# davidtweedle/gptq-svd

Hardware: AMD Instinct MI355X
Metric: weight-cols quantized/sec at d_in=4096 (higher is better)
Workload: dtype f64+f32; 1 GPU; single synthetic 4096x4096 Hessian per rank, full solver (eigh, rank rule, pivot order, U, 4-bit asym g128 quantize, pack); n=4096, m=4096, calib_rows=3072, rank_k=3058, threshold_method=energy, block_size=1024, parallelism=independent layer per rank x1

## Files before the change

### gptq-svd_amd/csrc/pivot.hip

```cpp
#include <algorithm>
#include <climits>
#include <cmath>
#include <cstdio>
#include <cstdlib>
#include <type_traits>
#include <utility>

#include "../../include/truncgptq.h"
#include "common.h"
#include "spin.h"
#include "gemm64.h"
#include "reduce.h"

namespace {

constexpr int PB = 32;
constexpr int PGMAX = 64;

struct PivWs {
  double *B;
  double *Hk;
  double *dsc;
  double *L;
  double *LT;
  double *part;
  int32_t *perm;
  int32_t *pos;
  unsigned *cnt;
  double *pp;
  double *bc;
  unsigned *flag;
  int32_t *sstate;
  int32_t *prow;
  double *pinv;
  double *Lpp;
  double *Hk2;
  int32_t *oidx;
};
constexpr int PPS = PB + 8;
static_assert(PGMAX * PPS % 256 == 0, "slot copy assumes whole rounds of 256 threads");

inline bool compact_pivot(int n) { return n <= 32768 && getenv("TG_PIVOT_OLD") == nullptr; }

template <class A>
void piv_layout(A &ar, int n, int k, PivWs *p) {
  PivWs d{};
  PivWs &q = p ? *p : d;
  auto take = [&](auto *&dst, size_t cnt) {
    using T = std::remove_reference_t<decltype(*dst)>;
    if constexpr (std::is_same_v<A, tg::Arena>) dst = ar.template take<T>(cnt);
    else ar.template take<T>(cnt);
  };
  auto take2m = [&](double *&dst, size_t cnt) {
    constexpr size_t AL = size_t(2) << 20;
    if constexpr (std::is_same_v<A, tg::Arena>) dst = ar.template take_aligned<double>(cnt, AL);
    else ar.template take_aligned<double>(cnt, AL);
  };
  take(q.B, size_t(k) * n);
  take(q.pp, size_t(2) * PGMAX * PPS);
  take(q.bc, PPS);
  take(q.flag, 16);
  take2m(q.Hk, size_t(n) * n);
  take(q.dsc, n);
  take(q.L, size_t(n) * k);
  take(q.LT, size_t(PB) * n);
  take(q.part, PGMAX * 2);
  take(q.perm, n);
  take(q.pos, n);
  take(q.cnt, 16);
  take(q.sstate, 16);
  take(q.prow, PB);
  take(q.pinv, PB);
  take(q.Lpp, PB * PB);
  take2m(q.Hk2, compact_pivot(n) ? size_t(n) * n : size_t(1));
  take(q.oidx, n);
}

__global__ void scale_rows_kernel(const double *__restrict__ Vh, int ldv, const double *__restrict__ S,
                                  int n, int k, double *__restrict__ B) {
  const int t = blockIdx.y;
  const double s = S[t];
  for (int c = blockIdx.x * blockDim.x + threadIdx.x; c < n; c += gridDim.x * blockDim.x)
    B[size_t(t) * n + c] = s * Vh[size_t(t) * ldv + c];
}

__device__ inline void argmax_publish(double bv, int bp, int i, int n, PivWs w) {
  __shared__ double sv[256];
  __shared__ int sp[256];
  __shared__ double vals[2];
  const int tid = threadIdx.x;
  sv[tid] = bv;
  sp[tid] = bp;
  __syncthreads();
  for (int off = 128; off > 0; off >>= 1) {
    if (tid < off) {
      const double ov = sv[tid + off];
      const int op = sp[tid + off];
      if (ov > sv[tid] || (ov == sv[tid] && op < sp[tid])) {
        sv[tid] = ov;
        sp[tid] = op;
      }
    }
    __syncthreads();
  }
  if (tid == 0) {
    vals[0] = sv[0];
    vals[1] = double(sp[0]);
  }
  __syncthreads();
  if (tg::publish_partials(vals, 2, w.part, w.cnt)) {
    if (tid < 64) {
      const int G = int(gridDim.x);
      double best = -INFINITY;
      int q = n;
      for (int g = tid; g < G; g += 64) {
        const double v = tg::load_partial(&w.part[g]);
        const int p = int(tg::load_partial(&w.part[G + g]));
        if (v > best || (v == best && p < q)) {
          best = v;
          q = p;
        }
      }
#pragma unroll
      for (int off = 32; off > 0; off >>= 1) {
        const double ov = __shfl_xor(best, off);
        const int op = __shfl_xor(q, off);
        if (ov > best || (ov == best && op < q)) {
          best = ov;
          q = op;
        }
      }
      if (tid == 0) {
        if (q < n && q != i) {
          const int a = w.perm[i], b = w.perm[q];
          w.perm[i] = b;
          w.perm[q] = a;
          w.pos[b] = i;
          w.pos[a] = q;
        }
        *w.cnt = 0u;
      }
    }
  }
}

__global__ __launch_bounds__(256) void piv_init_kernel(int n, PivWs w) {
  double bv = -INFINITY;
  int bp = n;
  for (int j = blockIdx.x * blockDim.x + threadIdx.x; j < n; j += gridDim.x * blockDim.x) {
    const double v = w.Hk[size_t(j) * n + j];
    w.dsc[j] = v;
    w.perm[j] = j;
    w.pos[j] = j;
    if (v > bv || (v == bv && j < bp)) {
      bv = v;
      bp = j;
    }
  }
// ... 249 lines not shown
    if (tid <= t) lrow[tid] = win[8 + tid];
    const int rowb = min(max(int(win[2]), 0), n - 1);
#pragma unroll
    for (int u = 0; u < RPT; ++u) hv[u] = w.Hk[size_t(rowb) * n + min(rows[u], n - 1)];
    const int a = permL[i + 1];
    __syncthreads();
    if (tid == 0 && q != i + 1) {
      permL[i + 1] = rowb;
      permL[q] = a;
      if (me == 0) {
        w.perm[i + 1] = rowb;
        w.perm[q] = a;
        w.pos[rowb] = i + 1;
        w.pos[a] = q;
      }
    }
#pragma unroll
    for (int u = 0; u < RPT; ++u) {
      if (rows[u] == rowb) posr[u] = i + 1;
      else if (rows[u] == a && q != i + 1) posr[u] = q;
    }
    dpiv = s_best;
    piv = rowb;
    __syncthreads();
  }
  const int pw = min(pe, k) - ps;
#pragma unroll
  for (int u = 0; u < RPT; ++u) {
    const int r = rows[u];
    if (r >= n) continue;
    w.dsc[r] = dsr[u];
#pragma unroll
    for (int l = 0; l < PB; ++l) {
      if (l < pw) {
        w.L[size_t(r) * k + ps + l] = lr[u][l];
        w.LT[size_t(l) * n + r] = lr[u][l];
      }
    }
  }
}

constexpr int SEL = 1024;
constexpr int SEL_LDS_N = 8192;

#ifdef TG_SEL_PHASES
__device__ unsigned long long g_selph[16];
#define SELT(i)                                                     \
  {                                                                 \
    const uint64_t tt = __builtin_amdgcn_s_memtime();               \
    if (i > 0 && threadIdx.x == 0) atomicAdd(g_selph + i - 1, tt - selt_last); \
    selt_last = tt;                                                 \
  }
#else
#define SELT(i)
#endif

__device__ inline unsigned long long dkey(double d) {
  return d > 0.0 ? static_cast<unsigned long long>(__double_as_longlong(d)) : 0ull;
}

__device__ __forceinline__ size_t hk_at(int a, int b, int n) {
  return size_t(max(a, b)) * n + min(a, b);
}

__device__ __forceinline__ unsigned hk_at32(int a, int b, int n) {
  return unsigned(max(a, b)) * unsigned(n) + unsigned(min(a, b));
}

constexpr int STH = 512;

constexpr int NLEV = 3;
constexpr int LEV_DOWN = 8;
enum { SS_LEV = 2, SS_RUN = 3, SS_PANELS = 4, SS_EARLY = 5, SS_ESC = 6, SS_NLEV = 7, SS_NEED = 10 };
static_assert(SS_NLEV + NLEV <= SS_NEED && SS_NEED + NLEV - 1 <= 16, "sstate words");

__device__ __forceinline__ bool lev_pays(int rem, int lost) {
  const int r = rem >> 6, extra_us = 35 + r * r / 94, gain_us = 14;
  return lost * extra_us < PB * gain_us;
}

struct SelPanel {
  int n, k, ps, pe, nset, bp, brow, bo, lev;
  bool adaptive;
  double tau, bv;
  const double *dS;
  const int32_t *pS;
  int *permL;
  const int *cand;
  double2 *rec;
  int *reco;
  double *lrow;
  unsigned long long t0;
};
template <int NW, int CP>
__device__ __forceinline__ void sel_steps(const SelPanel &sp, PivWs w,
                                          const double *__restrict__ Hc);

__device__ inline double vmax_d(double a, double b) {
  double r;
  asm("v_max_f64 %0, %1, %2" : "=v"(r) : "v"(a), "v"(b));
  return r;
}
__device__ inline double sel_pair_max(double x, bool half16) {
  const int lo = __double2loint(x), hi = __double2hiint(x);
  if (half16) {
    const auto l = __builtin_amdgcn_permlane16_swap(lo, lo, false, false);
    const auto h = __builtin_amdgcn_permlane16_swap(hi, hi, false, false);
    return vmax_d(__hiloint2double(h[0], l[0]), __hiloint2double(h[1], l[1]));
  }
  const auto l = __builtin_amdgcn_permlane32_swap(lo, lo, false, false);
  const auto h = __builtin_amdgcn_permlane32_swap(hi, hi, false, false);
  return vmax_d(__hiloint2double(h[0], l[0]), __hiloint2double(h[1], l[1]));
}
template <int CTRL>
__device__ inline double sel_dpp(double x) {
  return __hiloint2double(__builtin_amdgcn_update_dpp(0, __double2hiint(x), CTRL, 0xF, 0xF, false),
                          __builtin_amdgcn_update_dpp(0, __double2loint(x), CTRL, 0xF, 0xF, false));
}
__device__ inline double wave_max_d(double x) {
  x = sel_pair_max(x, false);
  x = sel_pair_max(x, true);
  x = vmax_d(x, sel_dpp<0x140>(x));
  x = vmax_d(x, sel_dpp<0x141>(x));
  x = vmax_d(x, sel_dpp<0x1B>(x));
  return vmax_d(x, sel_dpp<0xB1>(x));
}
template <int S>
__device__ inline int wave_min_stage(int x) {
  return min(x, partner<S>(x));
}
template <int NW>
__device__ inline void block_argmax_sel(double &v, int &p, int &r, int &o, double2 *rec,
                                        int *reco) {
  const double m = wave_max_d(v);
  const bool hold = v == m;
  const unsigned long long b = __ballot(hold);
  int L = __ffsll(static_cast<long long>(b)) - 1;
  if (__popcll(b) > 1 && m != -INFINITY) {
    int pp = hold ? p : INT_MAX;
    pp = wave_min_stage<0>(pp);
    pp = wave_min_stage<1>(pp);
    pp = wave_min_stage<2>(pp);
    pp = wave_min_stage<3>(pp);
    pp = wave_min_stage<4>(pp);
    pp = wave_min_stage<5>(pp);
    L = __ffsll(static_cast<long long>(__ballot(hold & (p == pp)))) - 1;
  }
  const int wp = __builtin_amdgcn_readlane(p, L), wr = __builtin_amdgcn_readlane(r, L);
  const int wo = __builtin_amdgcn_readlane(o, L);
  if ((threadIdx.x & 63) == 0) {
    rec[threadIdx.x >> 6] = make_double2(m, __hiloint2double(wp, wr));
    reco[threadIdx.x >> 6] = wo;
  }
  __syncthreads();
  double2 x[NW];
#pragma unroll
  for (int q = 0; q < NW; ++q) x[q] = rec[q];
  v = x[0].x;
#pragma unroll
  for (int q = 1; q < NW; ++q) v = vmax_d(v, x[q].x);
  p = INT_MAX;
  r = 0;
  o = 0;
#pragma unroll
  for (int q = 0; q < NW; ++q) {
    const int op = __double2hiint(x[q].y);
    const bool take = (x[q].x == v) & (op < p);
    p = take ? op : p;
    r = take ? __double2loint(x[q].y) : r;
    o = take ? reco[q] : o;
  }
}

constexpr int HPAD = 2048 + 64;
__device__ inline int hidx(int b) { return b + (b >> 5); }

__device__ inline void hist_add_agg(unsigned *hist, int bin, bool ok, int lane) {
  unsigned long long pend = __ballot(ok);
  while (pend) {
    const int L = __ffsll(static_cast<long long>(pend)) - 1;
    const int b = __builtin_amdgcn_readlane(bin, L);
    const unsigned long long same = __ballot(ok & (bin == b));
    if (lane == L) atomicAdd(&hist[hidx(b)], unsigned(__popcll(same)));
    pend &= ~same;
  }
}

__device__ inline void hist_scan(const unsigned *hist, int target, int *out) {
  const int lane = threadIdx.x & 63, blk = 63 - lane;
  int c[32];
#pragma unroll
  for (int j = 0; j < 32; ++j) c[j] = int(hist[blk * 33 + 31 - j]);
  int sum = 0;
#pragma unroll
  for (int j = 0; j < 32; ++j) sum += c[j];
  int pre = sum;
#pragma unroll
  for (int off = 1; off < 64; off <<= 1) {
    const int o = __shfl_up(pre, off);
    pre += lane >= off ? o : 0;
  }
  int acc = pre - sum;
  if (acc < target && pre >= target) {
    int cb = 0, cbefore = 0;
    bool found = false;
#pragma unroll
    for (int j = 0; j < 32; ++j) {
      const bool hit = !found & (acc + c[j] >= target);
      cb = hit ? j : cb;
      cbefore = hit ? acc : cbefore;
      found = found | hit;
      acc += c[j];
    }
    out[0] = blk * 32 + 31 - cb;
    out[1] = cbefore;
  }
}

__global__ __launch_bounds__(STH) void piv_sel_kernel(int n, int k, PivWs w,
                                                      const double *__restrict__ Hc, int flev) {
  extern __shared__ int permL[];
  __shared__ unsigned hist[HPAD];
  __shared__ int cand[SEL + 1];
  __shared__ double2 rec[STH / 64];
  __shared__ int reco[STH / 64];
  __shared__ double sv[STH / 64];
  __shared__ int scnt[STH / 64];
  __shared__ int sel[4];
  __shared__ double lrow[PB];
  const int tid = threadIdx.x, lane = tid & 63, wid = tid >> 6;
  const int ps = w.sstate[0];
  if (ps >= k) {
    if (tid == 0) w.sstate[1] = 0;
    return;
  }
  const int pe = min(ps + PB, k);
  const int lev = flev >= 0              ? flev
                  : !lev_pays(n - ps, 1) ? NLEV - 1
                                         : min(max(w.sstate[SS_LEV], 0), NLEV - 1);
  const int nsel = SEL >> (NLEV - 1 - lev);
#ifdef TG_SEL_PHASES
  uint64_t selt_last = 0;
#endif
  SELT(0)
  int nset, bp, brow, bo;
  double tau, bv;
  const double *dS;
  const int32_t *pS;
  const bool staged = n <= SEL_LDS_N;
  double *dsh = reinterpret_cast<double *>(permL + ((n + 1) & ~1));
  int *posh = reinterpret_cast<int *>(dsh + n);
  if (staged) {
    for (int r0 = tid; r0 < n; r0 += 8 * STH) {
      double dv[8];
      int pv[8], mv[8];
#pragma unroll
      for (int u = 0; u < 8; ++u) {
        const int r = min(r0 + u * STH, n - 1);
        dv[u] = w.dsc[r];
        pv[u] = w.pos[r];
        mv[u] = w.perm[r];
      }
#pragma unroll
      for (int u = 0; u < 8; ++u)
        if (r0 + u * STH < n) {
          dsh[r0 + u * STH] = dv[u];
          posh[r0 + u * STH] = pv[u];
          permL[r0 + u * STH] = mv[u];
        }
    }
  } else {
    for (int x = tid; x < n; x += STH) permL[x] = w.perm[x];
  }
  for (int x = tid; x < HPAD; x += STH) hist[x] = 0u;
  if (tid == 0) {
    sel[0] = -1;
    sel[2] = -1;
  }
  __syncthreads();
  SELT(9)
  dS = staged ? dsh : w.dsc;
  pS = staged ? posh : w.pos;
  int valid = 0;
  for (int r0 = tid; r0 < n; r0 += 8 * STH) {
    double dv[8];
    int pv[8];
#pragma unroll
    for (int u = 0; u < 8; ++u) {
      const int r = min(r0 + u * STH, n - 1);
      dv[u] = dS[r];
      pv[u] = pS[r];
    }
#pragma unroll
    for (int u = 0; u < 8; ++u) {
      const unsigned long long key = dkey(dv[u]);
      const bool ok = (r0 + u * STH < n) & (pv[u] >= ps) & (key != 0ull);
      valid += ok;
      hist_add_agg(hist, int(key >> 52), ok, lane);
    }
  }
#pragma unroll
  for (int off = 32; off > 0; off >>= 1) valid += __shfl_xor(valid, off);
  if (lane == 0) scnt[wid] = valid;
  __syncthreads();
  valid = 0;
#pragma unroll
  for (int q = 0; q < STH / 64; ++q) valid += scnt[q];
  SELT(10)
  if (valid > nsel) {
    if (wid == 0) hist_scan(hist, nsel, sel);
    __syncthreads();
    for (int x = tid; x < HPAD; x += STH) hist[x] = 0u;
    __syncthreads();
    const int b1 = sel[0];
    for (int r0 = tid; r0 < n; r0 += 8 * STH) {
      double dv[8];
      int pv[8];
#pragma unroll
      for (int u = 0; u < 8; ++u) {
        const int r = min(r0 + u * STH, n - 1);
        dv[u] = dS[r];
        pv[u] = pS[r];
      }
#pragma unroll
      for (int u = 0; u < 8; ++u) {
        const unsigned long long key = dkey(dv[u]);
        if ((r0 + u * STH < n) & (pv[u] >= ps) & (int(key >> 52) == b1))
          atomicAdd(&hist[hidx(int(key >> 41) & 2047)], 1u);
      }
    }
    __syncthreads();
    if (wid == 0) hist_scan(hist, nsel - sel[1], sel + 2);
    __syncthreads();
  }
  SELT(11)
  const int b1 = sel[0], b2 = sel[2];
  int mine = 0;
  tau = -INFINITY;
  bv = -INFINITY;
  bp = n;
  brow = 0;
  unsigned long long insm = 0ull;
  for (int r0 = tid, bi = 0; r0 < n; r0 += 8 * STH, bi += 8) {
    double dv[8];
    int pv[8];
#pragma unroll
    for (int u = 0; u < 8; ++u) {
      const int r = min(r0 + u * STH, n - 1);
      dv[u] = dS[r];
      pv[u] = pS[r];
    }
#pragma unroll
    for (int u = 0; u < 8; ++u) {
      const bool un = (r0 + u * STH < n) & (pv[u] >= ps);
      const unsigned long long key = dkey(dv[u]);
      const int d1 = int(key >> 52), d2 = int(key >> 41) & 2047;
      const bool ins = un & (key != 0ull) & ((b1 < 0) | (d1 > b1) | ((d1 == b1) & (d2 > b2)));
      mine += ins;
      insm |= static_cast<unsigned long long>(ins) << (bi + u);
      tau = (un & !ins) ? fmax(tau, dv[u]) : tau;
      const bool take = un & ((dv[u] > bv) | ((dv[u] == bv) & (pv[u] < bp)));
      bv = take ? dv[u] : bv;
      bp = take ? pv[u] : bp;
      brow = take ? r0 + u * STH : brow;
    }
  }
  {
    int pre = mine;
#pragma unroll
    for (int off = 1; off < 64; off <<= 1) {
      const int o = __shfl_up(pre, off);
      pre += lane >= off ? o : 0;
    }
    double t2 = tau;
#pragma unroll
    for (int off = 32; off > 0; off >>= 1) t2 = fmax(t2, __shfl_xor(t2, off));
    __syncthreads();
    if (lane == 63) scnt[wid] = pre;
    if (lane == 0) sv[wid] = t2;
    __syncthreads();
    int base = 0;
    tau = -INFINITY;
#pragma unroll
    for (int q = 0; q < STH / 64; ++q) {
      base += q < wid ? scnt[q] : 0;
      tau = fmax(tau, sv[q]);
    }
    int slot = base + pre - mine;
    for (int r0 = tid, bi = 0; r0 < n; r0 += 8 * STH, bi += 8) {
#pragma unroll
      for (int u = 0; u < 8; ++u) {
        const bool ins = (insm >> (bi + u)) & 1ull;
        cand[ins ? slot : SEL] = r0 + u * STH;
        slot += ins;
      }
    }
  }
  __syncthreads();
  SELT(12)
  nset = 0;
#pragma unroll
  for (int q = 0; q < STH / 64; ++q) nset += scnt[q];
  bo = bp - ps;
  block_argmax_sel<STH / 64>(bv, bp, brow, bo, rec, reco);
  SelPanel sp{n,   k,  ps, pe,    nset, bp,   brow, bo,   lev,  flev < 0,
              tau, bv, dS, pS,    permL, cand, rec,  reco, lrow,
#ifdef TG_SEL_PHASES
              selt_last
#else
              0
#endif
  };
  if (lev == NLEV - 1) {
    sel_steps<STH / 64, 2>(sp, w, Hc);
    return;
  }
  if (wid >= 4) return;
  if (lev == 1) sel_steps<4, 2>(sp, w, Hc);
  else sel_steps<4, 1>(sp, w, Hc);
}

template <int NW, int CP>
__device__ __forceinline__ void sel_steps(const SelPanel &sp, PivWs w,
                                          const double *__restrict__ Hc) {
  constexpr int NT = NW * 64;
  const int tid = threadIdx.x;
  const int n = sp.n, k = sp.k, ps = sp.ps, pe = sp.pe, nset = sp.nset;
  const double tau = sp.tau;
  const double *dS = sp.dS;
  const int32_t *pS = sp.pS;
  int *permL = sp.permL;
  const int *cand = sp.cand;
  double2 *rec = sp.rec;
  int *reco = sp.reco;
  double *lrow = sp.lrow;
#ifdef TG_SEL_PHASES
  uint64_t selt_last = sp.t0;
#endif
  const int ss_run = w.sstate[SS_RUN], ss_esc = w.sstate[SS_ESC], ss_panels = w.sstate[SS_PANELS],
            ss_early = w.sstate[SS_EARLY], ss_nlev = w.sstate[SS_NLEV + sp.lev],
            ss_need_up = w.sstate[SS_NEED + min(sp.lev, NLEV - 2)],
            ss_need_dn = w.sstate[SS_NEED + max(sp.lev - 1, 0)];
  int rc[CP], posc[CP], oc[CP];
  double dc[CP];
  bool done[CP];
  double lr[CP][PB];
#pragma unroll
  for (int u = 0; u < CP; ++u) {
    const int c = tid + u * NT;
    rc[u] = c < nset ? cand[c] : -1;
    posc[u] = rc[u] >= 0 ? pS[rc[u]] : n;
    oc[u] = rc[u] >= 0 ? posc[u] - ps : 0;
    dc[u] = rc[u] >= 0 ? dS[rc[u]] : -INFINITY;
    done[u] = rc[u] < 0;
#pragma unroll
    for (int l = 0; l < PB; ++l) lr[u][l] = 0.0;
  }
  int piv = sp.brow, q = sp.bp, opiv = sp.bo;
  double dpiv = sp.bv;
  int tdone = 0;
  SELT(1)
  bool active = true;
  auto step = [&]<int t>(std::integral_constant<int, t>) __attribute__((always_inline)) {
    const int i = ps + t;
    active = active && i < pe;
    if (!active) return;
    if (t > 0) {
      double v = -INFINITY;
      int p = n, r = -1, o = 0;
#pragma unroll
      for (int u = 0; u < CP; ++u) {
        const bool take = !done[u] & ((dc[u] > v) | ((dc[u] == v) & (posc[u] < p)));
        v = take ? dc[u] : v;
        p = take ? posc[u] : p;
        r = take ? rc[u] : r;
        o = take ? oc[u] : o;
      }
      SELT(4)
      block_argmax_sel<NW>(v, p, r, o, rec, reco);
      SELT(5)
      active = v > tau;
      if (!active) return;
      dpiv = v;
      q = p;
      piv = r;
      opiv = o;
    }
    double hv[CP];
#pragma unroll
    for (int u = 0; u < CP; ++u)
      hv[u] = Hc[hk_at32(opiv, oc[u], n)];
#pragma unroll
    for (int u = 0; u < CP; ++u)
      if (rc[u] == piv) {
#pragma unroll
        for (int l = 0; l < t; ++l) lrow[l] = lr[u][l];
      }
    if (tid == 0) {
      const int a = permL[i];
      if (q != i) {
        permL[i] = piv;
        permL[q] = a;
      }
      w.prow[t] = piv;
    }
    SELT(2)
    __syncthreads();
    SELT(3)
    const double ljj = sqrt(fmax(dpiv, 0.0));
    const double inv = ljj > 0.0 ? 1.0 / ljj : 0.0;
    if (tid == 0) w.pinv[t] = inv;
    if (tid <= t) w.Lpp[t * PB + tid] = tid < t ? lrow[tid] : ljj;
    double lrw[PB > 1 ? PB : 1];
#pragma unroll
    for (int l = 0; l < t; ++l) lrw[l] = lrow[l];
#pragma unroll
    for (int u = 0; u < CP; ++u) {
      const bool isp = rc[u] == piv;
      const bool upd = !done[u] & !isp;
      double v = hv[u];
#pragma unroll
      for (int l = 0; l < t; ++l) v = fma(-lr[u][l], lrw[l], v);
      const double lv = v * inv;
      lr[u][t] = isp ? ljj : (upd ? lv : lr[u][t]);
      dc[u] = upd ? fma(-lv, lv, dc[u]) : dc[u];
      const int pswap = ((posc[u] == i) & (q != i)) ? q : posc[u];
      posc[u] = isp ? i : (upd ? pswap : posc[u]);
      done[u] = done[u] | isp;
    }
    tdone = t + 1;
#ifdef TG_SEL_PHASES
    if (tid == 0) atomicAdd(g_selph + 15, 1ull);
#endif
  };
  [&]<int... Ts>(std::integer_sequence<int, Ts...>) __attribute__((always_inline)) {
    (step(std::integral_constant<int, Ts>{}), ...);
  }(std::make_integer_sequence<int, PB>{});
  SELT(6)
  __syncthreads();
  for (int x = ps + tid; x < n; x += NT) w.oidx[x - ps] = pS[permL[x]] - ps;
  __syncthreads();
  for (int x = tid; x < n; x += NT) {
    const int r = permL[x];
    w.perm[x] = r;
    w.pos[r] = x;
  }
  if (tid == 0) {
    w.sstate[0] = ps + tdone;
    w.sstate[1] = tdone;
    const bool early = tdone < PB && ps + tdone < k;
    if (sp.adaptive) {
      const bool shorted = early && !lev_pays(n - ps, pe - ps - tdone);
      int lev = sp.lev, run = shorted ? 0 : ss_run + 1;
      if (shorted && lev < NLEV - 1) {
        w.sstate[SS_NEED + lev] = min(2 * max(ss_need_up, LEV_DOWN), 1 << 20);
        ++lev;
        w.sstate[SS_ESC] = ss_esc + 1;
      } else if (lev > 0 && run >= max(ss_need_dn, LEV_DOWN)) {
        --lev;
        run = 0;
      }
      w.sstate[SS_LEV] = lev;
      w.sstate[SS_RUN] = run;
    }
    w.sstate[SS_PANELS] = ss_panels + 1;
    w.sstate[SS_EARLY] = ss_early + early;
    w.sstate[SS_NLEV + sp.lev] = ss_nlev + 1;
  }
}

template <int FT>
__global__ __launch_bounds__(FT) void piv_fill_kernel(int n, int k, PivWs w,
                                                      const double *__restrict__ Hc) {
  __shared__ double lpp[PB][PB + 1];
  __shared__ double pinv[PB];
  __shared__ int prow[PB], poi[PB];
  __shared__ double lst[FT][PB + 1];
  __shared__ int rst[FT];
  const int tid = threadIdx.x;
  const int tn = w.sstate[1];
  if (tn <= 0) return;
  const int ps = w.sstate[0] - tn, ps2 = ps + tn;
  for (int x = tid; x < PB * PB; x += FT) {
    const int i = x / PB, l = x % PB;
    lpp[i][l] = (i < tn && l <= i) ? w.Lpp[x] : 0.0;
  }
  if (tid < PB) {
    pinv[tid] = tid < tn ? w.pinv[tid] : 0.0;
    prow[tid] = tid < tn ? w.prow[tid] : -1;
    poi[tid] = tid < tn ? w.oidx[tid] : 0;
  }
  __syncthreads();
  const int x = ps + blockIdx.x * FT + tid;
  const bool valid = x < n;
  const int xc = valid ? x : n - 1;
  const int r = w.perm[xc], oi = w.oidx[xc - ps];
  double hv[PB];
#pragma unroll
  for (int i = 0; i < PB; ++i) hv[i] = i < tn ? Hc[hk_at(poi[i], oi, n)] : 0.0;
  double d = w.dsc[r];
  double lr[PB];
  bool done = false;
#pragma unroll
  for (int i = 0; i < PB; ++i) {
    double v = hv[i];
#pragma unroll
    for (int l = 0; l < i; ++l) v = fma(-lr[l], lpp[i][l], v);
    const double lv = v * pinv[i];
    const bool act = (i < tn) & !done, isp = prow[i] == r;
    lr[i] = act ? (isp ? lpp[i][i] : lv) : 0.0;
    d = (act & !isp) ? fma(-lv, lv, d) : d;
    done = done | (act & isp);
  }
  if (valid) w.dsc[r] = d;
#pragma unroll
  for (int l = 0; l < PB; ++l) {
    if (valid && x >= ps2) w.LT[size_t(l) * n + (x - ps2)] = lr[l];
    lst[tid][l] = lr[l];
  }
  rst[tid] = valid ? r : -1;
  __syncthreads();
  const int hw = tid >> 5, l = tid & 31;
  for (int t = hw; t < FT; t += FT / 32) {
    const int rr = rst[t];
    if (rr >= 0 && l < tn) w.L[size_t(rr) * k + ps + l] = lst[t][l];
  }
}

typedef double doublex4 __attribute__((ext_vector_type(4)));

__global__ __launch_bounds__(256) void syrk_compact_kernel(int n, PivWs w,
                                                           const double *__restrict__ Hc,
                                                           double *__restrict__ Hn) {
  __shared__ double li[PB][64], lj[PB][64];
  __shared__ int orow[64], ocol[64];
  const int tid = threadIdx.x;
  const int ps2 = w.sstate[0], tn = max(w.sstate[1], 0);
  const int nc = n - ps2;
  const int b = blockIdx.x;
  int I = int((sqrt(8.0 * b + 1.0) - 1.0) * 0.5);
  while ((I + 1) * (I + 2) / 2 <= b) ++I;
  while (I * (I + 1) / 2 > b) --I;
  const int J = b - I * (I + 1) / 2;
  const int i0 = 64 * I, j0 = 64 * J;
  if (i0 >= nc) return;
  if (tid < 64) {
    orow[tid] = w.oidx[tn + min(i0 + tid, nc - 1)];
  } else if (tid < 128) {
    ocol[tid - 64] = w.oidx[tn + min(j0 + tid - 64, nc - 1)];
  }
  for (int e = tid; e < PB * 64; e += 256) {
    const int l = e >> 6, c = e & 63;
    li[l][c] = w.LT[size_t(l) * n + min(i0 + c, nc - 1)];
    lj[l][c] = w.LT[size_t(l) * n + min(j0 + c, nc - 1)];
  }
  __syncthreads();
  const int lane = tid & 63, wid = tid >> 6, wm = wid >> 1, wn = wid & 1;
  const int lr = lane & 15, lk = lane >> 4;
  doublex4 acc[2][2];
#pragma unroll
  for (int ib = 0; ib < 2; ++ib)
#pragma unroll
    for (int jb = 0; jb < 2; ++jb)
#pragma unroll
      for (int q = 0; q < 4; ++q)
        acc[ib][jb][q] = Hc[hk_at(orow[wm * 32 + ib * 16 + lk + 4 * q], ocol[wn * 32 + jb * 16 + lr], n)];
#pragma unroll
  for (int kq = 0; kq < PB; kq += 4) {
    double af[2], bf[2];
#pragma unroll
    for (int ib = 0; ib < 2; ++ib) af[ib] = -li[kq + lk][wm * 32 + ib * 16 + lr];
#pragma unroll
    for (int jb = 0; jb < 2; ++jb) bf[jb] = lj[kq + lk][wn * 32 + jb * 16 + lr];
#pragma unroll
    for (int ib = 0; ib < 2; ++ib)
#pragma unroll
      for (int jb = 0; jb < 2; ++jb)
        acc[ib][jb] = __builtin_amdgcn_mfma_f64_16x16x4f64(af[ib], bf[jb], acc[ib][jb], 0, 0, 0);
  }
#pragma unroll
  for (int ib = 0; ib < 2; ++ib)
#pragma unroll
    for (int jb = 0; jb < 2; ++jb)
#pragma unroll
      for (int q = 0; q < 4; ++q) {
        const int rl = wm * 32 + ib * 16 + lk + 4 * q, cl = wn * 32 + jb * 16 + lr;
        const int gi = i0 + rl, gj = j0 + cl;
        if (gi < nc && gj < nc && gi >= gj) Hn[size_t(gi) * n + gj] = acc[ib][jb][q];
      }
}

__global__ __launch_bounds__(256, 2) void syrk_compact_p_kernel(int n, PivWs w,
                                                                const double *__restrict__ Hc,
                                                                double *__restrict__ Hn) {
  __shared__ double li[PB][64], lj[PB][64];
  const int tid = threadIdx.x;
  const int ps2 = w.sstate[0], tn = max(w.sstate[1], 0);
  const int nc = n - ps2;
  if (nc <= 0) return;
  const int ntile = tg::cdiv(nc, 64), tiles = ntile * (ntile + 1) / 2;
  const int lane = tid & 63, wid = tid >> 6, wm = wid >> 1, wn = wid & 1;
  const int lr = lane & 15, lk = lane >> 4;
  auto tile_ij = [&](int b, int &i0, int &j0) __attribute__((always_inline)) {
// ... 17 lines not shown
      __attribute__((always_inline)) {
#pragma unroll
    for (int ib = 0; ib < 2; ++ib)
#pragma unroll
      for (int jb = 0; jb < 2; ++jb)
#pragma unroll
        for (int q = 0; q < 4; ++q) o[ib][jb][q] = Hc[hk_at(ro[ib][q], co[jb], n)];
  };
  int b = blockIdx.x;
  if (b >= tiles) return;
  int ro[2][4], co[2];
  double old[2][2][4], nold[2][2][4];
  load_idx(b, ro, co);
  load_old(ro, co, old);
  const int G = int(gridDim.x);
  if (b + G < tiles) load_idx(b + G, ro, co);
  for (; b < tiles; b += G) {
    int i0, j0;
    tile_ij(b, i0, j0);
    __syncthreads();
    double lv[8][2];
#pragma unroll
    for (int u = 0; u < 8; ++u) {
      const int e = tid + u * 256, l = e >> 6, c = e & 63;
      lv[u][0] = w.LT[size_t(l) * n + min(i0 + c, nc - 1)];
      lv[u][1] = w.LT[size_t(l) * n + min(j0 + c, nc - 1)];
    }
    __builtin_amdgcn_sched_barrier(0);
    const bool more = b + G < tiles;
    if (more) load_old(ro, co, nold);
    __builtin_amdgcn_sched_barrier(0);
#pragma unroll
    for (int u = 0; u < 8; ++u) {
      const int e = tid + u * 256, l = e >> 6, c = e & 63;
      li[l][c] = lv[u][0];
      lj[l][c] = lv[u][1];
    }
    __syncthreads();
    if (b + 2 * G < tiles) load_idx(b + 2 * G, ro, co);
    doublex4 acc[2][2];
#pragma unroll
    for (int ib = 0; ib < 2; ++ib)
#pragma unroll
      for (int jb = 0; jb < 2; ++jb)
#pragma unroll
        for (int q = 0; q < 4; ++q) acc[ib][jb][q] = old[ib][jb][q];
#pragma unroll
    for (int kq = 0; kq < PB; kq += 4) {
      double af[2], bf[2];
#pragma unroll
      for (int ib = 0; ib < 2; ++ib) af[ib] = -li[kq + lk][wm * 32 + ib * 16 + lr];
#pragma unroll
      for (int jb = 0; jb < 2; ++jb) bf[jb] = lj[kq + lk][wn * 32 + jb * 16 + lr];
#pragma unroll
      for (int ib = 0; ib < 2; ++ib)
#pragma unroll
        for (int jb = 0; jb < 2; ++jb)
          acc[ib][jb] = __builtin_amdgcn_mfma_f64_16x16x4f64(af[ib], bf[jb], acc[ib][jb], 0, 0, 0);
    }
#pragma unroll
    for (int ib = 0; ib < 2; ++ib)
#pragma unroll
      for (int jb = 0; jb < 2; ++jb)
#pragma unroll
        for (int q = 0; q < 4; ++q) {
          const int rl = wm * 32 + ib * 16 + lk + 4 * q, cl = wn * 32 + jb * 16 + lr;
          const int gi = i0 + rl, gj = j0 + cl;
          if (gi < nc && gj < nc && gi >= gj) Hn[size_t(gi) * n + gj] = acc[ib][jb][q];
        }
#pragma unroll
    for (int ib = 0; ib < 2; ++ib)
#pragma unroll
      for (int jb = 0; jb < 2; ++jb)
#pragma unroll
        for (int q = 0; q < 4; ++q) old[ib][jb][q] = nold[ib][jb][q];
  }
}

__global__ __launch_bounds__(256) void piv_init2_kernel(int n, PivWs w) {
  for (int j = blockIdx.x * blockDim.x + threadIdx.x; j < n; j += gridDim.x * blockDim.x) {
    w.dsc[j] = w.Hk[size_t(j) * n + j];
    w.perm[j] = j;
    w.pos[j] = j;
  }
  if (blockIdx.x == 0 && threadIdx.x < 16) w.sstate[threadIdx.x] = 0;
}

__global__ void rx_gather_kernel(int n, int k, PivWs w, double *__restrict__ Rx, int ldr,
                                 int64_t *__restrict__ perm64) {
  const int t = blockIdx.y;
  for (int j = blockIdx.x * blockDim.x + threadIdx.x; j < n; j += gridDim.x * blockDim.x) {
    const int r = w.perm[j];
    if (t == 0) perm64[j] = r;
    if (Rx) Rx[size_t(t) * ldr + j] = j >= t ? w.L[size_t(r) * k + t] : 0.0;
  }
}

}

extern "C" size_t tg_pivot_workspace_size(int n, int k) {
  tg::Sizer s;
  piv_layout(s, n, k, nullptr);
  return s.off + 256;
}

static int pivot_core_sel(hipStream_t st, PivWs &w, int n, int k) {
#ifdef TG_SEL_PHASES
  static bool reg = false;
  if (!reg) {
    reg = true;
    atexit([] {
      unsigned long long h[16];
      (void)hipMemcpyFromSymbol(h, HIP_SYMBOL(g_selph), sizeof(h));
      const char *nm[12] = {"sel:argmax+cand", "head", "barrier2", "compute+wargmax", "blockargmax",
                            "?", "tail", "?", "sel:stage", "sel:count", "sel:radix", "sel:compact"};
      fprintf(stderr, "sel phases (cycles, thread 0):");
      for (int q = 0; q < 12; ++q) fprintf(stderr, " %s %.3g", nm[q], double(h[q]));
      fprintf(stderr, " steps %llu", h[15]);
      fprintf(stderr, "\n");
    });
  }
#endif
  hipLaunchKernelGGL(piv_init2_kernel, dim3(std::min(64, tg::cdiv(n, 256))), dim3(256), 0, st, n, w);
  TG_LAUNCHED();
  const size_t lds = sizeof(int) * size_t((n + 1) & ~1) +
                     (n <= SEL_LDS_N ? (sizeof(double) + sizeof(int)) * size_t(n) : 0);
  if (lds > 48 * 1024)
    TG_HIP(hipFuncSetAttribute((const void *)piv_sel_kernel,
                               hipFuncAttributeMaxDynamicSharedMemorySize, int(lds)));
  const char *ps = getenv("TG_SYR2K_PERSIST");
  const bool persist = !(ps && ps[0] == '0');
  const tg::XcdInfo xi = tg::xcd_info();
  const int ncu = std::max(1, xi.xcds * xi.cus_per_xcd);
  const double *hc = w.Hk;
  double *hn = w.Hk2;
  auto schur_compact = [&](int rows) -> hipError_t {
    const int nt = tg::cdiv(rows, 64);
    if (persist)
      hipLaunchKernelGGL(syrk_compact_p_kernel, dim3(std::min(nt * (nt + 1) / 2, 2 * ncu)),
                         dim3(256), 0, st, n, w, hc, hn);
    else
      hipLaunchKernelGGL(syrk_compact_kernel, dim3(nt * (nt + 1) / 2), dim3(256), 0, st, n, w, hc,
                         hn);
    const hipError_t e = hipGetLastError();
    double *t = const_cast<double *>(hc);
    hc = hn;
    hn = t;
    return e;
  };
  int flev = -1;
  if (const char *pl = getenv("TG_PIV_LEVEL")) {
    const int v = atoi(pl);
    flev = v == 256 ? 0 : v == 512 ? 1 : v == 1024 ? 2 : -1;
  }
  int done = 0;
  int pend_rows = 0;
  for (int round = 0;; ++round) {
    if (round > 4 * (k / PB + 2)) {
      tg::set_error("pivot order: no progress after %d rounds (%d of %d steps)", round, done, k);
      return int(hipErrorUnknown);
    }
    const int P = tg::cdiv(k - done, PB);
    for (int p = 0; p < P; ++p) {
      const int rows = n - (done + p);
      if (pend_rows > 0) TG_HIP(schur_compact(pend_rows));
      auto tok = tg::prof_begin(st, tg::PROF_PIVSTEP, 8.0 * double(n) * PB * 3, 0.0);
      hipLaunchKernelGGL(piv_sel_kernel, dim3(1), dim3(STH), lds, st, n, k, w, hc, flev);
      hipLaunchKernelGGL(piv_fill_kernel<64>, dim3(tg::cdiv(rows, 64)), dim3(64), 0, st, n, k, w, hc);
      tg::prof_end(st, tok);
      TG_LAUNCHED();
      pend_rows = rows;
    }
    int32_t h = 0;
    TG_HIP(hipMemcpyAsync(&h, w.sstate, sizeof(int32_t), hipMemcpyDeviceToHost, st));
    TG_HIP(hipStreamSynchronize(st));
    if (h >= k) break;
    pend_rows = n - (done + P - 1);
    done = h;
  }
  if (const char *pst = getenv("TG_PIV_STATS"); pst && pst[0] == '1') {
    int32_t h[16];
    TG_HIP(hipMemcpyAsync(h, w.sstate, sizeof(h), hipMemcpyDeviceToHost, st));
    TG_HIP(hipStreamSynchronize(st));
    fprintf(stderr,
            "pivot stats: n=%d k=%d panels=%d early=%d escalations=%d level256=%d level512=%d "
            "level1024=%d\n",
            n, k, h[SS_PANELS], h[SS_EARLY], h[SS_ESC], h[SS_NLEV], h[SS_NLEV + 1], h[SS_NLEV + 2]);
  }
  return 0;
}

static int pivot_core(hipStream_t st, PivWs &w, int n, int k, int64_t *perm, double *Rx, int ldr) {
  if (compact_pivot(n)) {
    const int e = pivot_core_sel(st, w, n, k);
    if (e != 0) return e;
    hipLaunchKernelGGL(rx_gather_kernel, dim3(tg::cdiv(n, 256) < 16 ? tg::cdiv(n, 256) : 16, k),
                       dim3(256), 0, st, n, k, w, Rx, ldr, perm);
    TG_LAUNCHED();
    return 0;
  }
  const int g0 = std::min(PGMAX, tg::cdiv(n, 256));
  hipLaunchKernelGGL(piv_init_kernel, dim3(g0), dim3(256), 0, st, n, w);
  TG_LAUNCHED();
  const int G = std::max(1, std::min(PGMAX, tg::cdiv(n, 256)));
  const int rpt = tg::cdiv(n, G * 256);
  const bool persistent = rpt <= 2 && n <= 32768 && getenv("TG_PIVOT_STEPWISE") == nullptr;
  if (persistent && n * sizeof(int) > 64 * 1024) {
    TG_HIP(hipFuncSetAttribute((const void *)piv_panel_kernel<1>,
                               hipFuncAttributeMaxDynamicSharedMemorySize, int(n * sizeof(int))));
    TG_HIP(hipFuncSetAttribute((const void *)piv_panel_kernel<2>,
                               hipFuncAttributeMaxDynamicSharedMemorySize, int(n * sizeof(int))));
  }
  TG_HIP(hipMemsetAsync(w.flag, 0, 16 * sizeof(unsigned), st));
  for (int ps = 0; ps < k; ps += PB) {
    const int pe = std::min(ps + PB, k);
    if (persistent) {
      auto tok = tg::prof_begin(st, tg::PROF_PIVSTEP, 8.0 * double(n) * (pe - ps) * 3, 0.0);
      const size_t lds = sizeof(int) * size_t(n);
      TG_HIP(hipMemsetAsync(w.flag + 4, 0, 9 * sizeof(unsigned), st));
      const int grid = 8 * G;
      if (rpt == 1)
        hipLaunchKernelGGL(piv_panel_kernel<1>, dim3(grid), dim3(256), lds, st, n, k, ps, pe, G,
                           unsigned(G) * unsigned(ps), w);
      else
        hipLaunchKernelGGL(piv_panel_kernel<2>, dim3(grid), dim3(256), lds, st, n, k, ps, pe, G,
                           unsigned(G) * unsigned(ps), w);
      tg::prof_end(st, tok);
      TG_LAUNCHED();
    } else {
      for (int i = ps; i < pe; ++i) {
        auto tok = tg::prof_begin(st, tg::PROF_PIVSTEP, 8.0 * double(n - i) * (i - ps + 3), 0.0);
        hipLaunchKernelGGL(piv_step_kernel, dim3(G), dim3(256), 0, st, n, k, i, ps, w);
        tg::prof_end(st, tok);
        TG_LAUNCHED();
      }
    }
    if (pe < k)
      TG_HIP(tg::dsyrk_tn(st, n, pe - ps, -1.0, w.LT, n, 1.0, w.Hk, n));
  }
  hipLaunchKernelGGL(rx_gather_kernel, dim3(tg::cdiv(n, 256) < 16 ? tg::cdiv(n, 256) : 16, k),
                     dim3(256), 0, st, n, k, w, Rx, ldr, perm);
  TG_LAUNCHED();
  return 0;
}

extern "C" int tg_pivoted_factor(void *stream, const double *Vh, int ldv, const double *S, int n,
                                 int k, int64_t *perm, double *Rx, int ldr, void *ws,
                                 size_t ws_bytes) {
  TG_ARG(Vh, 2, "null Vh");
  TG_ARG(ldv >= n, 3, "ldv < n");
  TG_ARG(S, 4, "null S");
// ... 50 lines not shown
```

Before: 70220 cols/s.

## Stream pivot steps to concurrent worker blocks during selection kernel

The pivot selection kernel now launches extra worker blocks alongside the single selector block. A publisher wave writes each pivot step (row, scale, Lpp row) to global memory with agent-scope atomics. Workers poll a sequence word and compute the L panel rows and diagonal updates while selection is still running, so the fill work overlaps the serial selection instead of following it. The fill kernel then skips row blocks the workers already finished. This adds spin-wait polling, a time budget with fallback, and cross-block memory-ordering risk.

```diff
diff --git a/gptq-svd_amd/csrc/pivot.hip b/gptq-svd_amd/csrc/pivot.hip
--- a/gptq-svd_amd/csrc/pivot.hip
+++ b/gptq-svd_amd/csrc/pivot.hip
@@ -36,6 +36,10 @@
   double *Lpp;
   double *Hk2;
   int32_t *oidx;
+  unsigned long long *strm;
+  int32_t *ppoi;
+  int32_t *pq;
+  int32_t *fdone;
 };
 constexpr int PPS = PB + 8;
 static_assert(PGMAX * PPS % 256 == 0, "slot copy assumes whole rounds of 256 threads");
@@ -74,6 +78,10 @@
   take(q.Lpp, PB * PB);
   take2m(q.Hk2, compact_pivot(n) ? size_t(n) * n : size_t(1));
   take(q.oidx, n);
+  take(q.strm, 2);
+  take(q.ppoi, PB);
+  take(q.pq, PB);
+  take(q.fdone, size_t(tg::cdiv(n, 64)));
 }
 
 __global__ void scale_rows_kernel(const double *__restrict__ Vh, int ldv, const double *__restrict__ S,
@@ -489,6 +497,7 @@
 struct SelPanel {
   int n, k, ps, pe, nset, bp, brow, bo, lev;
   bool adaptive;
+  bool pub;
   double tau, bv;
   const double *dS;
   const int32_t *pS;
@@ -535,6 +544,27 @@
 template <int S>
 __device__ inline int wave_min_stage(int x) {
   return min(x, partner<S>(x));
+}
+template <int NW>
+__device__ inline void sel_merge(double &v, int &p, int &r, int &o, const double2 *rec,
+                                 const int *reco) {
+  double2 x[NW];
+#pragma unroll
+  for (int q = 0; q < NW; ++q) x[q] = rec[q];
+  v = x[0].x;
+#pragma unroll
+  for (int q = 1; q < NW; ++q) v = vmax_d(v, x[q].x);
+  p = INT_MAX;
+  r = 0;
+  o = 0;
+#pragma unroll
+  for (int q = 0; q < NW; ++q) {
+    const int op = __double2hiint(x[q].y);
+    const bool take = (x[q].x == v) & (op < p);
+    p = take ? op : p;
+    r = take ? __double2loint(x[q].y) : r;
+    o = take ? reco[q] : o;
+  }
 }
 template <int NW>
 __device__ inline void block_argmax_sel(double &v, int &p, int &r, int &o, double2 *rec,
@@ -560,23 +590,7 @@
     reco[threadIdx.x >> 6] = wo;
   }
   __syncthreads();
-  double2 x[NW];
-#pragma unroll
-  for (int q = 0; q < NW; ++q) x[q] = rec[q];
-  v = x[0].x;
-#pragma unroll
-  for (int q = 1; q < NW; ++q) v = vmax_d(v, x[q].x);
-  p = INT_MAX;
-  r = 0;
-  o = 0;
-#pragma unroll
-  for (int q = 0; q < NW; ++q) {
-    const int op = __double2hiint(x[q].y);
-    const bool take = (x[q].x == v) & (op < p);
-    p = take ? op : p;
-    r = take ? __double2loint(x[q].y) : r;
-    o = take ? reco[q] : o;
-  }
+  sel_merge<NW>(v, p, r, o, rec, reco);
 }
 
 constexpr int HPAD = 2048 + 64;
@@ -624,9 +638,224 @@
   }
 }
 
+__device__ __forceinline__ void piv_scale(double dpiv, double &ljj, double &inv) {
+  ljj = sqrt(fmax(dpiv, 0.0));
+  inv = ljj > 0.0 ? 1.0 / ljj : 0.0;
+}
+
+typedef __attribute__((address_space(1))) double pv_f64;
+typedef __attribute__((address_space(1))) int32_t pv_i32;
+typedef __attribute__((address_space(1))) unsigned long long pv_u64;
+__device__ __forceinline__ void st_sc1d(double *p, double v) {
+  __hip_atomic_store((pv_f64 *)p, v, __ATOMIC_RELAXED, __HIP_MEMORY_SCOPE_AGENT);
+}
+__device__ __forceinline__ double ld_sc1d(const double *p) {
+  return __hip_atomic_load((pv_f64 *)const_cast<double *>(p), __ATOMIC_RELAXED,
+                           __HIP_MEMORY_SCOPE_AGENT);
+}
+__device__ __forceinline__ void st_sc1i(int32_t *p, int v) {
+  __hip_atomic_store((pv_i32 *)p, v, __ATOMIC_RELAXED, __HIP_MEMORY_SCOPE_AGENT);
+}
+__device__ __forceinline__ int ld_sc1i(const int32_t *p) {
+  return __hip_atomic_load((pv_i32 *)const_cast<int32_t *>(p), __ATOMIC_RELAXED,
+                           __HIP_MEMORY_SCOPE_AGENT);
+}
+__device__ __forceinline__ void st_sc1u(unsigned long long *p, unsigned long long v) {
+  __hip_atomic_store((pv_u64 *)p, v, __ATOMIC_RELAXED, __HIP_MEMORY_SCOPE_AGENT);
+}
+__device__ __forceinline__ unsigned long long ld_sc1u(const unsigned long long *p) {
+  return __hip_atomic_load((pv_u64 *)const_cast<unsigned long long *>(p), __ATOMIC_RELAXED,
+                           __HIP_MEMORY_SCOPE_AGENT);
+}
+
+constexpr unsigned long long SW_ENDED = 64ull, SW_NOSTREAM = 128ull, SW_STEPS = 63ull;
+static_assert(PB <= int(SW_STEPS), "step count field");
+__device__ __forceinline__ unsigned long long sw_word(unsigned seq, int ps) {
+  return (static_cast<unsigned long long>(seq) << 32) |
+         (static_cast<unsigned long long>(ps & 0xffff) << 16);
+}
+
+template <int NW>
+__device__ __forceinline__ void sel_publish(const SelPanel &sp, PivWs w, unsigned seq) {
+  const int lane = threadIdx.x & 63;
+  const int ps = sp.ps, pe = sp.pe;
+  const unsigned long long base = sw_word(seq, ps);
+  int piv = sp.brow, q = sp.bp, opiv = sp.bo;
+  double dpiv = sp.bv;
+  int tdone = 0;
+  for (int t = 0; t < PB; ++t) {
+    if (ps + t >= pe) break;
+    if (t > 0) {
+      __syncthreads();
+      double v;
+      int p, r, o;
+      sel_merge<NW>(v, p, r, o, sp.rec, sp.reco);
+      v = __hiloint2double(__builtin_amdgcn_readfirstlane(__double2hiint(v)),
+                           __builtin_amdgcn_readfirstlane(__double2loint(v)));
+      asm volatile("s_waitcnt vmcnt(0)" ::: "memory");
+      if (lane == 0) st_sc1u(w.strm, base | static_cast<unsigned long long>(t));
+      if (!(v > sp.tau)) break;
+      dpiv = v;
+      q = __builtin_amdgcn_readfirstlane(p);
+      piv = __builtin_amdgcn_readfirstlane(r);
+      opiv = __builtin_amdgcn_readfirstlane(o);
+    }
+    __syncthreads();
+    double ljj, inv;
+    piv_scale(dpiv, ljj, inv);
+    if (lane <= t) st_sc1d(w.Lpp + t * PB + lane, lane < t ? sp.lrow[lane] : ljj);
+    if (lane == 0) {
+      st_sc1i(w.prow + t, piv);
+      st_sc1i(w.ppoi + t, opiv);
+      st_sc1i(w.pq + t, q);
+      st_sc1d(w.pinv + t, inv);
+    }
+    tdone = t + 1;
+  }
+  asm volatile("s_waitcnt vmcnt(0)" ::: "memory");
+  if (lane == 0) st_sc1u(w.strm, base | SW_ENDED | static_cast<unsigned long long>(tdone));
+  __syncthreads();
+  asm volatile("s_waitcnt vmcnt(0)" ::: "memory");
+  __syncthreads();
+}
+
+constexpr int WK_ROWS = 64;
+constexpr size_t WK_LDS = sizeof(double) * (PB * PB + PB) + sizeof(int) * 3 * PB;
+
+__device__ inline unsigned long long strm_wait(const unsigned long long *word, unsigned seq,
+                                               int have, uint64_t t0, unsigned budget) {
+  unsigned long long v;
+  for (;;) {
+    const unsigned long long x = ld_sc1u(word);
+    v = (static_cast<unsigned long long>(
+             __builtin_amdgcn_readfirstlane(static_cast<unsigned>(x >> 32)))
+         << 32) |
+        __builtin_amdgcn_readfirstlane(static_cast<unsigned>(x));
+    if (static_cast<unsigned>(v >> 32) == seq &&
+        ((v & (SW_ENDED | SW_NOSTREAM)) != 0ull || int(v & SW_STEPS) > have))
+      break;
+    if (__builtin_amdgcn_s_memrealtime() - t0 > budget) {
+      v = 0ull;
+      break;
+    }
+    __builtin_amdgcn_s_sleep(4);
+  }
+  __builtin_amdgcn_fence(__ATOMIC_ACQUIRE, "wavefront");
+  return v;
+}
+
+__device__ __forceinline__ void piv_stream_worker(int n, int k, PivWs w,
+                                                  const double *__restrict__ Hc, unsigned seq,
+                                                  unsigned budget, char *smem) {
+  double *lpl = reinterpret_cast<double *>(smem);
+  double *pinv_s = lpl + PB * PB;
+  int *prow_s = reinterpret_cast<int *>(pinv_s + PB);
+  int *poi_s = prow_s + PB, *pq_s = poi_s + PB;
+  const int lane = threadIdx.x, c = int(blockIdx.x) - 1;
+  if (seq == 0u || budget == 0u) return;
+  const uint64_t t0 = __builtin_amdgcn_s_memrealtime();
+  const unsigned long long hdr = strm_wait(w.strm, seq, -1, t0, budget);
+  if (hdr == 0ull || (hdr & SW_NOSTREAM) != 0ull) return;
+  const int ps = int((hdr >> 16) & 0xffffull);
+  if (ps + WK_ROWS * c >= n) return;
+  const int x0 = ps + WK_ROWS * c + lane;
+  const bool valid = x0 < n;
+  const int xc = valid ? x0 : n - 1;
+  const int rl = w.perm[xc];
+  const int r = valid ? rl : -1;
+  const int oi = xc - ps;
+  double d = w.dsc[rl];
+  asm volatile("s_waitcnt vmcnt(0)" ::: "memory");
+  {
+    const unsigned long long x = ld_sc1u(w.strm);
+    const bool stale = static_cast<unsigned>(x >> 32) != seq || (x & SW_ENDED) != 0ull;
+    if (__builtin_amdgcn_readfirstlane(int(stale))) return;
+  }
+  double lr[PB];
+#pragma unroll
+  for (int l = 0; l < PB; ++l) lr[l] = 0.0;
+  bool done = false;
+  int pos = x0;
+  int have = 0;
+  for (;;) {
+    const unsigned long long pw = strm_wait(w.strm, seq, have, t0, budget);
+    if (pw == 0ull) return;
+    const int s = min(int(pw & SW_STEPS), PB);
+    if (s > have) {
+      if (lane >= have && lane < s) {
+        const int pr = ld_sc1i(w.prow + lane), po = ld_sc1i(w.ppoi + lane), pq = ld_sc1i(w.pq + lane);
+        const double pi = ld_sc1d(w.pinv + lane);
+        prow_s[lane] = pr;
+        poi_s[lane] = min(max(po, 0), n - ps - 1);
+        pq_s[lane] = pq;
+        pinv_s[lane] = pi;
+      }
+      for (int e0 = have * PB; e0 < s * PB; e0 += 4 * 64) {
+        double v[4];
+#pragma unroll
+        for (int u = 0; u < 4; ++u) {
+          const int e = e0 + lane + 64 * u;
+          v[u] = e < s * PB ? ld_sc1d(w.Lpp + e) : 0.0;
+        }
+#pragma unroll
+        for (int u = 0; u < 4; ++u) {
+          const int e = e0 + lane + 64 * u;
+          if (e < s * PB) lpl[e] = v[u];
+        }
+      }
+      __syncthreads();
+#pragma unroll
+      for (int j = 0; j < PB; ++j)
+        if (j >= have && j < s) lr[j] = Hc[hk_at(poi_s[j], oi, n)];
+#pragma unroll
+      for (int t = 0; t < PB; ++t) {
+        if (t >= have && t < s) {
+          const double *lp = lpl + t * PB;
+          double v = lr[t];
+#pragma unroll
+          for (int l = 0; l < t; ++l) v = fma(-lr[l], lp[l], v);
+          const double lv = v * pinv_s[t];
+          const bool act = !done, isp = prow_s[t] == r;
+          lr[t] = act ? (isp ? lp[t] : lv) : 0.0;
+          d = (act & !isp) ? fma(-lv, lv, d) : d;
+          const int i = ps + t, q = pq_s[t];
+          pos = (act & isp) ? i : ((pos == i) & (q != i)) ? q : pos;
+          done = done | (act & isp);
+          if ((t & 3) == 3 && valid) {
+            double *dst = w.L + size_t(r) * k + ps + (t - 3);
+#pragma unroll
+            for (int u = 0; u < 4; ++u) dst[u] = lr[t - 3 + u];
+          }
+        }
+      }
+      have = s;
+    }
+    if ((pw & SW_ENDED) != 0ull) break;
+  }
+  const int tn = have, ps2 = ps + tn;
+  if (tn <= 0) return;
+  if (valid) w.dsc[r] = d;
+#pragma unroll
+  for (int l = 0; l < PB; ++l) {
+    if (valid && pos >= ps2 && pos < n) w.LT[size_t(l) * n + (pos - ps2)] = lr[l];
+    if (valid && l >= (tn & ~3) && l < tn) w.L[size_t(r) * k + ps + l] = lr[l];
+  }
+  if (lane == 0) {
+    w.fdone[c] = int(seq);
+    (void)__hip_atomic_fetch_add((pv_u64 *)(w.strm + 1), 1ull, __ATOMIC_RELAXED,
+                                 __HIP_MEMORY_SCOPE_AGENT);
+  }
+}
+
 __global__ __launch_bounds__(STH) void piv_sel_kernel(int n, int k, PivWs w,
-                                                      const double *__restrict__ Hc, int flev) {
+                                                      const double *__restrict__ Hc, int flev,
+                                                      unsigned seq, unsigned budget) {
   extern __shared__ int permL[];
+  if (blockIdx.x != 0) {
+    if (threadIdx.x < 64)
+      piv_stream_worker(n, k, w, Hc, seq, budget, reinterpret_cast<char *>(permL));
+    return;
+  }
   __shared__ unsigned hist[HPAD];
   __shared__ int cand[SEL + 1];
   __shared__ double2 rec[STH / 64];
@@ -638,7 +867,10 @@
   const int tid = threadIdx.x, lane = tid & 63, wid = tid >> 6;
   const int ps = w.sstate[0];
   if (ps >= k) {
-    if (tid == 0) w.sstate[1] = 0;
+    if (tid == 0) {
+      w.sstate[1] = 0;
+      if (seq != 0u) st_sc1u(w.strm, sw_word(seq, ps) | SW_NOSTREAM | SW_ENDED);
+    }
     return;
   }
   const int pe = min(ps + PB, k);
@@ -646,6 +878,11 @@
                   : !lev_pays(n - ps, 1) ? NLEV - 1
                                          : min(max(w.sstate[SS_LEV], 0), NLEV - 1);
   const int nsel = SEL >> (NLEV - 1 - lev);
+  const bool pub = seq != 0u && lev < NLEV - 1;
+  if (seq != 0u && tid == 4 * 64) {
+    st_sc1u(w.strm + 1, 0ull);
+    st_sc1u(w.strm, sw_word(seq, ps) | (pub ? 0ull : SW_NOSTREAM | SW_ENDED));
+  }
 #ifdef TG_SEL_PHASES
   uint64_t selt_last = 0;
 #endif
@@ -810,7 +1047,7 @@
   for (int q = 0; q < STH / 64; ++q) nset += scnt[q];
   bo = bp - ps;
   block_argmax_sel<STH / 64>(bv, bp, brow, bo, rec, reco);
-  SelPanel sp{n,   k,  ps, pe,    nset, bp,   brow, bo,   lev,  flev < 0,
+  SelPanel sp{n,   k,  ps, pe,    nset, bp,   brow, bo,   lev,  flev < 0, pub,
               tau, bv, dS, pS,    permL, cand, rec,  reco, lrow,
 #ifdef TG_SEL_PHASES
               selt_last
@@ -822,7 +1059,10 @@
     sel_steps<STH / 64, 2>(sp, w, Hc);
     return;
   }
-  if (wid >= 4) return;
+  if (wid >= 4) {
+    if (pub && wid == 4) sel_publish<4>(sp, w, seq);
+    return;
+  }
   if (lev == 1) sel_steps<4, 2>(sp, w, Hc);
   else sel_steps<4, 1>(sp, w, Hc);
 }
@@ -909,15 +1149,17 @@
         permL[i] = piv;
         permL[q] = a;
       }
-      w.prow[t] = piv;
+      if (!sp.pub) w.prow[t] = piv;
     }
     SELT(2)
     __syncthreads();
     SELT(3)
-    const double ljj = sqrt(fmax(dpiv, 0.0));
-    const double inv = ljj > 0.0 ? 1.0 / ljj : 0.0;
-    if (tid == 0) w.pinv[t] = inv;
-    if (tid <= t) w.Lpp[t * PB + tid] = tid < t ? lrow[tid] : ljj;
+    double ljj, inv;
+    piv_scale(dpiv, ljj, inv);
+    if (!sp.pub) {
+      if (tid == 0) w.pinv[t] = inv;
+      if (tid <= t) w.Lpp[t * PB + tid] = tid < t ? lrow[tid] : ljj;
+    }
     double lrw[PB > 1 ? PB : 1];
 #pragma unroll
     for (int l = 0; l < t; ++l) lrw[l] = lrow[l];
@@ -978,7 +1220,8 @@
 
 template <int FT>
 __global__ __launch_bounds__(FT) void piv_fill_kernel(int n, int k, PivWs w,
-                                                      const double *__restrict__ Hc) {
+                                                      const double *__restrict__ Hc,
+                                                      unsigned seq) {
   __shared__ double lpp[PB][PB + 1];
   __shared__ double pinv[PB];
   __shared__ int prow[PB], poi[PB];
@@ -986,11 +1229,22 @@
   __shared__ int rst[FT];
   const int tid = threadIdx.x;
   const int tn = w.sstate[1];
+  const unsigned long long wdone = seq != 0u ? w.strm[1] : 0ull;
   if (tn <= 0) return;
   const int ps = w.sstate[0] - tn, ps2 = ps + tn;
-  for (int x = tid; x < PB * PB; x += FT) {
-    const int i = x / PB, l = x % PB;
-    lpp[i][l] = (i < tn && l <= i) ? w.Lpp[x] : 0.0;
+  if (seq != 0u && wdone == static_cast<unsigned long long>(tg::cdiv(n - ps, 64))) return;
+  const int x = ps + blockIdx.x * FT + tid;
+  const bool valid = x < n;
+  const int xc = valid ? x : n - 1;
+  const int r = w.perm[xc], oi = w.oidx[xc - ps];
+  bool todo = valid;
+  if (seq != 0u) {
+    todo = valid && unsigned(w.fdone[oi >> 6]) != seq;
+    if (!__syncthreads_or(todo)) return;
+  }
+  for (int e = tid; e < PB * PB; e += FT) {
+    const int i = e / PB, l = e % PB;
+    lpp[i][l] = (i < tn && l <= i) ? w.Lpp[e] : 0.0;
   }
   if (tid < PB) {
     pinv[tid] = tid < tn ? w.pinv[tid] : 0.0;
@@ -998,10 +1252,6 @@
     poi[tid] = tid < tn ? w.oidx[tid] : 0;
   }
   __syncthreads();
-  const int x = ps + blockIdx.x * FT + tid;
-  const bool valid = x < n;
-  const int xc = valid ? x : n - 1;
-  const int r = w.perm[xc], oi = w.oidx[xc - ps];
   double hv[PB];
 #pragma unroll
   for (int i = 0; i < PB; ++i) hv[i] = i < tn ? Hc[hk_at(poi[i], oi, n)] : 0.0;
@@ -1019,13 +1269,13 @@
     d = (act & !isp) ? fma(-lv, lv, d) : d;
     done = done | (act & isp);
   }
-  if (valid) w.dsc[r] = d;
+  if (todo) w.dsc[r] = d;
 #pragma unroll
   for (int l = 0; l < PB; ++l) {
-    if (valid && x >= ps2) w.LT[size_t(l) * n + (x - ps2)] = lr[l];
+    if (todo && x >= ps2) w.LT[size_t(l) * n + (x - ps2)] = lr[l];
     lst[tid][l] = lr[l];
   }
-  rst[tid] = valid ? r : -1;
+  rst[tid] = todo ? r : -1;
   __syncthreads();
   const int hw = tid >> 5, l = tid & 31;
   for (int t = hw; t < FT; t += FT / 32) {
@@ -1209,7 +1459,9 @@
     w.dsc[j] = w.Hk[size_t(j) * n + j];
     w.perm[j] = j;
     w.pos[j] = j;
-  }
+    if (j < tg::cdiv(n, 64)) w.fdone[j] = 0;
+  }
+  if (blockIdx.x == 0 && threadIdx.x < 2) w.strm[threadIdx.x] = 0ull;
   if (blockIdx.x == 0 && threadIdx.x < 16) w.sstate[threadIdx.x] = 0;
 }
 
@@ -1250,8 +1502,14 @@
 #endif
   hipLaunchKernelGGL(piv_init2_kernel, dim3(std::min(64, tg::cdiv(n, 256))), dim3(256), 0, st, n, w);
   TG_LAUNCHED();
-  const size_t lds = sizeof(int) * size_t((n + 1) & ~1) +
-                     (n <= SEL_LDS_N ? (sizeof(double) + sizeof(int)) * size_t(n) : 0);
+  const char *sv = getenv("TG_PIV_STREAM");
+  const bool stream = !(sv && sv[0] == '0');
+  unsigned budget = 200000u;
+  if (const char *sb = getenv("TG_PIV_STREAM_BUDGET")) budget = unsigned(strtoul(sb, nullptr, 10));
+  unsigned seq = 0;
+  const size_t lds = std::max(sizeof(int) * size_t((n + 1) & ~1) +
+                                  (n <= SEL_LDS_N ? (sizeof(double) + sizeof(int)) * size_t(n) : 0),
+                              stream ? WK_LDS : size_t(0));
   if (lds > 48 * 1024)
     TG_HIP(hipFuncSetAttribute((const void *)piv_sel_kernel,
                                hipFuncAttributeMaxDynamicSharedMemorySize, int(lds)));
@@ -1292,8 +1550,12 @@
       const int rows = n - (done + p);
       if (pend_rows > 0) TG_HIP(schur_compact(pend_rows));
       auto tok = tg::prof_begin(st, tg::PROF_PIVSTEP, 8.0 * double(n) * PB * 3, 0.0);
-      hipLaunchKernelGGL(piv_sel_kernel, dim3(1), dim3(STH), lds, st, n, k, w, hc, flev);
-      hipLaunchKernelGGL(piv_fill_kernel<64>, dim3(tg::cdiv(rows, 64)), dim3(64), 0, st, n, k, w, hc);
+      const int nwork = stream ? std::min(ncu - 1, tg::cdiv(rows, WK_ROWS)) : 0;
+      if (stream) ++seq;
+      hipLaunchKernelGGL(piv_sel_kernel, dim3(1 + nwork), dim3(STH), lds, st, n, k, w, hc, flev, seq,
+                         budget);
+      hipLaunchKernelGGL(piv_fill_kernel<64>, dim3(tg::cdiv(rows, 64)), dim3(64), 0, st, n, k, w, hc,
+                         seq);
       tg::prof_end(st, tok);
       TG_LAUNCHED();
       pend_rows = rows;
```

Measured after the change: 71790 cols/s, median of 6. 2.2% higher.
